# libnxz/power-gzip

Measured on AMD Instinct MI355X. Metric: GiB/s uncompressed in (deflate), real-data corpus in 64 KiB blocks, exact dynamic-Huffman table per block, higher is better.
Workload: dtype u8

## Files before the change

### power-gzip_amd/csrc/nxz_lz77.hip

```cpp
#include <hip/hip_runtime.h>
#include <type_traits>
#include <stdint.h>
#include "nxz_device.h"
#include "nxz_dhtgen_dev.h"
#include "nxz_dict.h"

__device__ unsigned long long *nxz_lz77_prof_buf = nullptr;
#define NXZ_GLOBAL NXZ_GLOBAL_AS
#ifdef NXZ_LZ77_PROF
#define WPROF_BEGIN() unsigned long long wp_ = prof ? clock64() : 0
#define WPROF_END(idx) do { if (prof) { const unsigned long long now_ = clock64(); wacc[(idx) - 16] += now_ - wp_; wp_ = now_; } } while (0)
#define PROF(idx) do { if (prof) { if (t == 0) { unsigned long long now_ = clock64(); profacc[idx] += (uint32_t)(now_ - tprev); tprev = now_; } } } while (0)
#define PCOUNT(idx, n) do { if (prof && lane == 0) atomicAdd(&profacc[idx], (uint32_t)(n)); } while (0)
#ifdef NXZ_LZ77_PROF2
#define PC2(idx, n) do { if (prof && lane == 0) __hip_atomic_fetch_add(&prof[32 + (idx)], (unsigned long long)(n), __ATOMIC_RELAXED, __HIP_MEMORY_SCOPE_AGENT); } while (0)
#else
#define PC2(idx, n) do { } while (0)
#endif
#else
#define PC2(idx, n) do { } while (0)
#define PCOUNT(idx, n) do { } while (0)
#define WPROF_BEGIN() do { } while (0)
#define WPROF_END(idx) do { } while (0)
#define PROF(idx) do { } while (0)
#endif

namespace nxzl77 {

constexpr int NT = 1024;
constexpr int HBITS = 13;
constexpr uint32_t HSIZE = 1u << HBITS;
constexpr uint32_t PTILE = 16384;
constexpr uint32_t PSEG = 16;
constexpr uint32_t NSEG = PTILE / PSEG;
constexpr uint32_t ETILE = 2048;
constexpr uint32_t LAZY_MAX = 32;
constexpr uint32_t MAXMATCH = 258;
constexpr uint32_t WINDOW = 32768;
constexpr uint32_t OPEN2 = 24;
constexpr uint32_t NOHASH = 0xFFFFu;
constexpr uint32_t SECOND_MIN_TOKENS = 3072;
constexpr uint32_t TEXT_HIGH_DIV = 16;
#ifndef NXZ_GROUP_ROUNDS
#define NXZ_GROUP_ROUNDS 24
#endif
#ifndef NXZ_GROUP_MIN
#define NXZ_GROUP_MIN 2
#endif
#ifndef NXZ_GROUP_GATE
#define NXZ_GROUP_GATE 3
#endif
constexpr uint32_t GROUP_ROUNDS = NXZ_GROUP_ROUNDS;
constexpr uint32_t GROUP_GATE = NXZ_GROUP_GATE;
constexpr uint32_t GROUP_MIN = NXZ_GROUP_MIN;
constexpr uint32_t C2_STRIDE = PTILE + 1024;

constexpr uint32_t OFF_IN    = 0;
constexpr uint32_t OFF_HEAD  = 65536 + 32;
constexpr uint32_t OFF_CAND  = OFF_HEAD + HSIZE * 4 + 256;
constexpr uint32_t OFF_MLEN  = OFF_CAND + PTILE * 2;
constexpr uint32_t OFF_SBITS = OFF_MLEN + PTILE;
constexpr uint32_t OFF_MBITS = OFF_SBITS + PTILE / 8;
constexpr uint32_t OFF_X     = OFF_MBITS + PTILE / 8;
constexpr uint32_t OFF_ENTRY = OFF_X + NSEG * 2;
constexpr uint32_t OFF_BITS  = OFF_ENTRY + NSEG * 2;
#ifndef NXZ_LQ_CAP
#define NXZ_LQ_CAP 128
#define NXZ_LQ_MIN 64
#endif
#ifndef NXZ_XQ_CAP
#define NXZ_XQ_CAP 120
#define NXZ_XQ_MIN 56
#endif
constexpr uint32_t LQ_CAP = NXZ_LQ_CAP, LQ_MIN = NXZ_LQ_MIN, XQ_CAP = NXZ_XQ_CAP, XQ_MIN = NXZ_XQ_MIN;
static_assert(LQ_MIN + 64 <= LQ_CAP && XQ_MIN + 64 <= XQ_CAP && LQ_CAP % 8 == 0 && XQ_CAP % 8 == 0, "a batch of 64 must fit behind what waits");
constexpr uint32_t BITS_BYTES = 16 * (LQ_CAP + XQ_CAP) * 2 + 2096 - NSEG * 4 < ETILE * 2 + 64 ? ETILE * 2 + 64 : 16 * (LQ_CAP + XQ_CAP) * 2 + 2096 - NSEG * 4;
constexpr uint32_t OFF_LQ    = OFF_X;
constexpr uint32_t OFF_DQ    = OFF_LQ;
constexpr uint32_t OFF_XQ    = OFF_LQ + 16 * LQ_CAP * 2;
constexpr uint32_t OFF_EB    = OFF_XQ + 16 * XQ_CAP * 2;
constexpr uint32_t EBO       = 32;
static_assert(OFF_EB % 16 == 0 && OFF_EB + 2096 <= OFF_BITS + BITS_BYTES, "match-phase carve");
constexpr uint32_t OFF_SCAN  = OFF_BITS + BITS_BYTES;
constexpr uint32_t OFF_HIST  = OFF_SCAN + 256;
constexpr uint32_t OFF_MISC  = OFF_HIST + 316 * 4;
constexpr uint32_t OFF_PROF  = OFF_MISC + 64;
constexpr uint32_t LDS_BYTES = OFF_PROF + 80;
static_assert(LDS_BYTES <= 163840, "LDS budget");
static_assert(OFF_HEAD % 16 == 0 && OFF_BITS % 16 == 0 && OFF_SCAN % 16 == 0, "alignment");

enum { M_NREC = 0, M_TOK0 = 1, M_HIGH = 2, M_DQ = 3, M_PROGRESS = 4, M_TICKET = 5, M_DEFER = 6, M_NEXT = 7, M_KEEP = 8, M_DEFER2 = 9, M_PREV = 12, M_JOBNO = 13 };
static_assert(M_TICKET == M_PROGRESS + 1 && M_DEFER == M_PROGRESS + 2, "cleared together");

__device__ __forceinline__ uint32_t lds_ld32(const uint32_t *inw, uint32_t r)
{
	uint32_t a = inw[r >> 2], b = inw[(r >> 2) + 1];
	return __builtin_amdgcn_alignbyte(b, a, r & 3);
}

__device__ __forceinline__ uint32_t hash4(uint32_t v) { return (v * 0x9E3779B1u) >> (32 - HBITS); }

__device__ __forceinline__ uint32_t equal16(const uint32_t *inw, uint32_t a, uint32_t b)
{
	const uint32_t aw = a >> 2, bw = b >> 2, as = a & 3, bs = b & 3;
	const uint32_t a0 = inw[aw], a1 = inw[aw + 1], a2 = inw[aw + 2], a3 = inw[aw + 3], a4 = inw[aw + 4];
	const uint32_t b0 = inw[bw], b1 = inw[bw + 1], b2 = inw[bw + 2], b3 = inw[bw + 3], b4 = inw[bw + 4];
	const uint32_t x0 = __builtin_amdgcn_alignbyte(a1, a0, as) ^ __builtin_amdgcn_alignbyte(b1, b0, bs);
	const uint32_t x1 = __builtin_amdgcn_alignbyte(a2, a1, as) ^ __builtin_amdgcn_alignbyte(b2, b1, bs);
	const uint32_t x2 = __builtin_amdgcn_alignbyte(a3, a2, as) ^ __builtin_amdgcn_alignbyte(b3, b2, bs);
	const uint32_t x3 = __builtin_amdgcn_alignbyte(a4, a3, as) ^ __builtin_amdgcn_alignbyte(b4, b3, bs);
	uint32_t n = 16;
	if (x3) n = 12 + ((uint32_t)__builtin_ctz(x3) >> 3);
	if (x2) n = 8 + ((uint32_t)__builtin_ctz(x2) >> 3);
	if (x1) n = 4 + ((uint32_t)__builtin_ctz(x1) >> 3);
	if (x0) n = (uint32_t)__builtin_ctz(x0) >> 3;
	return n;
}

__device__ __forceinline__ uint32_t gf_mul(uint32_t a, uint32_t b)
{
	uint32_t r = 0;
#pragma unroll 8
	for (int i = 0; i < 32; i++) {
		r ^= (b & 0x80000000u) ? a : 0;
		a = (a >> 1) ^ ((a & 1) ? 0xedb88320u : 0);
		b <<= 1;
	}
	return r;
}

constexpr uint32_t cgf_mul(uint32_t a, uint32_t b)
{
	uint32_t r = 0;
	for (int i = 0; i < 32; i++) {
		if (b & 0x80000000u) r ^= a;
		a = (a >> 1) ^ ((a & 1) ? 0xedb88320u : 0);
		b <<= 1;
	}
	return r;
}
struct PowTab { uint32_t v[1024]; };
constexpr PowTab make_pow()
{
	PowTab p{};
	uint32_t m = 0x00800000u;
	for (int k = 0; k < 6; k++) m = cgf_mul(m, m);
	p.v[0] = 0x80000000u;
	for (int i = 1; i < 1024; i++) p.v[i] = cgf_mul(p.v[i - 1], m);
	return p;
}
__device__ const PowTab CRC_POW = make_pow();
struct Pow8Tab { uint32_t v[65]; };
constexpr Pow8Tab make_pow8()
{
	Pow8Tab p{};
	p.v[0] = 0x80000000u;
	for (int i = 1; i <= 64; i++) p.v[i] = cgf_mul(p.v[i - 1], 0x00800000u);
	return p;
}
__device__ const Pow8Tab CRC_POW8 = make_pow8();

__device__ __forceinline__ uint32_t wave_incl_scan(uint32_t v, int lane)
{
#pragma unroll
	for (int o = 1; o < 64; o <<= 1) {
		uint32_t u = __shfl_up(v, o, 64);
		if (lane >= o) v += u;
	}
	return v;
}
// ... 274 lines not shown
	__syncthreads();
	uint32_t *w_ = win0 + par * (WW + 2);
	if (n == 0) {
		const uint32_t nfull = base_bits >> 5;
		for (uint32_t i = te; i < nfull; i += ENT)
			if (wordbase + i < cap_words) dstw[wordbase + i] = w_[i];
		const uint32_t keep = w_[nfull];
		__syncthreads();
		if (te == 0) w_[0] = keep;
		wordbase += nfull;
		base_bits &= 31;
		__syncthreads();
	}
	if (te == 0) {
		const uint32_t lt = lltab[256];
		uint32_t cc = 0;
		if (wordbase > cap_words) cc = NXZ_CC_TARGET_SPACE;
		if ((lt >> 16) == 0) cc = NXZ_CC_MISSING_CODE;
		if (tb->status) cc = NXZ_CC_INVALID_DHT;
		const uint64_t acc = (uint64_t)w_[0] | ((uint64_t)(lt & 0xffff) << base_bits);
		const uint32_t bits = base_bits + (lt >> 16);
		const uint64_t totbits = (uint64_t)wordbase * 32 + bits;
		const uint32_t tpbc = (uint32_t)((totbits + 7) >> 3);
		if (tpbc > job.dst_cap) cc = cc ? cc : NXZ_CC_TARGET_SPACE;
		if (cc != NXZ_CC_TARGET_SPACE && (uint64_t)wordbase * 4 + (bits + 7) / 8 <= job.dst_cap) {
			NXZ_GLOBAL uint8_t *o = (NXZ_GLOBAL uint8_t *)job.dst + (size_t)wordbase * 4;
			for (uint32_t b = 0; b < (bits + 7) / 8; b++) o[b] = (uint8_t)(acc >> (8 * b));
		}
		if (cc == 0 && tpbc > total) cc = NXZ_CC_TPBC_GT_SPBC;
		nxz_batch_result_t *r = results + bid;
		r->cc = cc;
		r->tpbc = cc == NXZ_CC_TARGET_SPACE ? 0 : tpbc;
		r->tebc = (uint32_t)(totbits & 7);
		r->sfbt = 0;
	}
}

__device__ __forceinline__ void post(uint8_t *lds, const nxz_batch_job_t *__restrict__ jobs, NXZ_GLOBAL uint8_t *scratch, nxz_batch_result_t *__restrict__ results,
				     bool have_cur, uint32_t cur_slot, uint32_t prev_plus1, uint32_t prev_slot, const int t)
{
	const NXZ_GLOBAL uint8_t *tabs = scratch + table_off(gridDim.x);
	const bool have_prev = prev_plus1 != 0;
	uint32_t nprev = 0;
	if (have_prev) {
		const uint32_t sl = jobs[prev_plus1 - 1].src_len, hl = jobs[prev_plus1 - 1].hist_len;
		nprev = sl - (hl < sl ? hl : sl);
	}
	nprev = (uint32_t)__builtin_amdgcn_readfirstlane((int)nprev);
	if (t < 64) {
		Credit cr{ have_prev ? encode_barriers(nprev) : 0u };
		if (have_cur) {
			uint32_t *hist = (uint32_t *)(lds + OFF_HIST);
			if (t == 0) hist[256] = 1;
			__builtin_amdgcn_fence(__ATOMIC_ACQ_REL, "wavefront");
			__builtin_amdgcn_wave_barrier();
			__builtin_amdgcn_s_setprio(3);
			nxzd::dhtgen_wave(lds + P_DHT, (const uint32_t *)hist, (nxz_dht_prepared_t *)(tabs + ((size_t)blockIdx.x * 2 + cur_slot) * sizeof(nxz_dht_prepared_t)),
					  (nxz_batch_dht_t *)nullptr, t, cr);
			__builtin_amdgcn_s_setprio(0);
		}
		while (cr.n) cr();
	} else if (have_prev) {
		encode(lds, jobs, prev_plus1 - 1, scratch + ((size_t)blockIdx.x * 2 + prev_slot) * NXZ_TOK_STRIDE,
		       (const NXZ_GLOBAL nxz_dht_prepared_t *)(tabs + ((size_t)blockIdx.x * 2 + prev_slot) * sizeof(nxz_dht_prepared_t)), results, t - 64);
	}
	__builtin_amdgcn_fence(__ATOMIC_RELEASE, "workgroup");
	__syncthreads();
	__builtin_amdgcn_fence(__ATOMIC_ACQUIRE, "workgroup");
}
}

template <bool COUNT, bool FUSED, bool GEN, bool DICT>
__device__ __forceinline__ void lz77_body(const nxz_batch_job_t *__restrict__ jobs,
					  uint8_t *__restrict__ tokens, uint16_t *__restrict__ cand2,
					  nxz_batch_result_t *__restrict__ results,
					  uint32_t *__restrict__ counts, uint32_t njobs, uint32_t *__restrict__ next_job,
					  const uint8_t *__restrict__ dict)
{
	__shared__ __attribute__((aligned(16))) uint8_t lds[LDS_BYTES];
	uint32_t *inw = (uint32_t *)(lds + OFF_IN);
	uint32_t *head = (uint32_t *)(lds + OFF_HEAD);
	uint16_t *cand = (uint16_t *)(lds + OFF_CAND);
	uint8_t *mlen = lds + OFF_MLEN;
	uint16_t *X = (uint16_t *)(lds + OFF_X);
	uint16_t *entry = (uint16_t *)(lds + OFF_ENTRY);
	uint32_t *sbits = (uint32_t *)(lds + OFF_SBITS);
	uint32_t *mbits = (uint32_t *)(lds + OFF_MBITS);
	uint32_t *tokbits = sbits;
	uint32_t *litbits = mbits;
	uint8_t *mark = lds + OFF_SBITS;
	uint16_t *jump = (uint16_t *)(lds + OFF_MBITS);
	uint32_t *bitbuf = (uint32_t *)(lds + OFF_BITS);
	uint32_t *scan = (uint32_t *)(lds + OFF_SCAN);
	uint32_t *hist = (uint32_t *)(lds + OFF_HIST);
	uint32_t *misc = (uint32_t *)(lds + OFF_MISC);
#ifdef NXZ_LZ77_PROF
	uint32_t *profacc = (uint32_t *)(lds + OFF_PROF);
#endif

#ifdef NXZ_LZ77_PROF
	NXZ_GLOBAL unsigned long long *prof = (NXZ_GLOBAL unsigned long long *)nxz_lz77_prof_buf;
#endif
	if constexpr (GEN) {
		if (threadIdx.x == 0) { misc[M_PREV] = 0; misc[M_JOBNO] = 0; }
		__syncthreads();
	}
	for (uint32_t bid = blockIdx.x; bid < njobs;) {
	if (next_job && threadIdx.x == 0) misc[M_NEXT] = gridDim.x + atomicAdd(next_job, 1u);
	int tid_ = threadIdx.x;
	asm volatile("" : "+v"(tid_));
	const int t = tid_, lane = t & 63, wave = t >> 6;
#ifdef NXZ_LZ77_PROF
	unsigned long long tprev = prof ? clock64() : 0;
	unsigned long long wacc[4] = { 0, 0, 0, 0 };
#endif
	const nxz_batch_job_t job = jobs[bid];
	const uint32_t total = job.src_len;
	const uint32_t h = job.hist_len < total ? job.hist_len : total;
	const uint32_t n = total - h;
	const uint32_t end = total;
	const NXZ_GLOBAL uint8_t *src = (const NXZ_GLOBAL uint8_t *)job.src;
	const uint32_t K1 = n ? (end - 1) >> 6 : 0;
	const uint32_t pw_slice = CRC_POW.v[(1022 - t) & 1023];
	const uint32_t pw_tail = CRC_POW8.v[n ? end - K1 * 64 : 0];

	{
		typedef uint32_t v4u __attribute__((ext_vector_type(4)));
		const NXZ_GLOBAL v4u *s4 = (const NXZ_GLOBAL v4u *)src;
		v4u *d4 = (v4u *)inw;
		uint32_t nfull = total >> 4;
		if constexpr (DICT) {
			const NXZ_GLOBAL v4u *w4 = (const NXZ_GLOBAL v4u *)dict;
			const uint32_t hq = h >> 4;
			for (uint32_t i = t; i < nfull; i += NT) d4[i] = i < hq ? w4[i] : s4[i];
		} else
		for (uint32_t i = t; i < nfull; i += NT) d4[i] = s4[i];
		uint32_t base = nfull << 4;
		for (uint32_t i = base + t; i < base + 48 && i < 65536 + 32; i += NT)
			lds[OFF_IN + i] = i < total ? src[i] : 0;
	}
	for (uint32_t i = t; i < HSIZE; i += NT) head[i] = 0;
	if (t < 316) hist[t] = 0;
	if (t < 16 && t != M_NEXT && !(GEN && (t == M_PREV || t == M_JOBNO))) misc[t] = FUSED && t == M_KEEP ? 3u : 0u;
#ifdef NXZ_LZ77_PROF
	if (t < 20) profacc[t] = 0;
#endif
	{
		uint32_t c = t & 255;
		for (int k = 0; k < 8 * ((t >> 8) + 1); k++) c = (c >> 1) ^ ((c & 1) ? 0xedb88320u : 0);
		bitbuf[t] = c;
	}
	__syncthreads();
	PROF(0);

	uint32_t out_crc, out_adler;
	{
		uint32_t *T = bitbuf;
		const uint32_t initx = job.in_crc ^ 0xffffffffu;
		const int sidx = (int)t - 1023 + (int)K1;
		uint32_t crc = 0, s1 = 0, sj = 0;
		if (n && sidx >= (int)(h >> 6)) {
			const uint4 *sp = (const uint4 *)(lds + OFF_IN + (uint32_t)sidx * 64);
			uint4 q[4] = { sp[0], sp[1], sp[2], sp[3] };
			uint32_t *w = (uint32_t *)q;
			const uint32_t a0 = (uint32_t)sidx * 64;
			if (a0 < h || a0 + 64 > end) {
#pragma unroll
				for (int k = 0; k < 16; k++)
					if (a0 + 4 * k < h || a0 + 4 * k + 4 > end) w[k] = 0;
			}
			uint32_t S = 0, Wt = 0;
#pragma unroll
			for (int k = 0; k < 16; k++) {
				S = __builtin_amdgcn_udot4(w[k], 0x01010101u, S, false);
				Wt = __builtin_amdgcn_udot4(w[k], 0x03020100u + 0x04040404u * k, Wt, false);
			}
			s1 = S;
			sj = S * (n + h - a0) - Wt;
			const uint32_t kfirst = a0 < h ? (h - a0) >> 2 : 0;
			if (a0 <= h && h < a0 + 64) {
				if (h + 4 <= end) {
					if (kfirst == 0) w[0] ^= initx;
					if (kfirst == 4) w[4] ^= initx;
					if (kfirst == 8) w[8] ^= initx;
					if (kfirst == 12) w[12] ^= initx;
				}
			}
			const uint32_t nd = a0 + 64 <= end ? 16 : (end - a0) >> 2;
#pragma unroll
			for (int k = 0; k < 16; k++) {
				const uint32_t c = crc ^ w[k];
				const uint32_t nc = T[768 + (c & 0xff)] ^ T[512 + ((c >> 8) & 0xff)] ^ T[256 + ((c >> 16) & 0xff)] ^ T[c >> 24];
				crc = (uint32_t)k < nd ? nc : crc;
			}
			if (t == 1023 && (end & 3)) {
				const uint32_t a = end & ~3u, nb = end & 3, i = a - h;
				const uint32_t v = inw[a >> 2] & ((1u << (8 * nb)) - 1);
				uint32_t b0 = v & 0xff, b1 = (v >> 8) & 0xff, b2 = (v >> 16) & 0xff;
				s1 += b0 + b1 + b2;
				sj += (b0 + b1 + b2) * (n - i) - (b1 + 2 * b2);
				if (i == 0) crc ^= initx;
				for (uint32_t k = 0; k < nb; k++) crc = T[(crc ^ (v >> (8 * k))) & 0xff] ^ (crc >> 8);
			}
		}
		uint32_t tailcrc = 0;
		if (t == 1023) { tailcrc = crc; crc = 0; }
		else if (crc) crc = gf_mul(crc, pw_slice);
		for (int o = 32; o > 0; o >>= 1) crc ^= __shfl_down(crc, o, 64);
		if (lane == 0) scan[wave] = crc;
		if (t == 1023) scan[50] = tailcrc;
		uint32_t a1 = s1, a2 = sj % 65521u;
		for (int o = 32; o > 0; o >>= 1) {
			a1 += __shfl_down(a1, o, 64);
			a2 += __shfl_down(a2, o, 64);
		}
		if (lane == 0) { scan[16 + wave] = a1; scan[32 + wave] = a2 % 65521u; }
		__syncthreads();
		if (wave == 0) {
			uint32_t c = lane < 16 ? scan[lane] : 0;
			uint32_t b1 = lane < 16 ? scan[16 + lane] : 0, b2 = lane < 16 ? scan[32 + lane] : 0;
			for (int o = 8; o > 0; o >>= 1) {
				c ^= __shfl_down(c, o, 64);
				b1 += __shfl_down(b1, o, 64);
				b2 += __shfl_down(b2, o, 64);
			}
			if (lane == 0) {
				c = n ? gf_mul(c, pw_tail) ^ scan[50] : initx;
				uint32_t ia = job.in_adler & 0xffff, ib = job.in_adler >> 16;
// ... 491 lines not shown
					lqn += (uint32_t)__popcll(m);
					PCOUNT(13, __popcll(m));
#endif
					__builtin_amdgcn_wave_barrier();
					WPROF_END(17);
					while (lqn >= (last ? 1u : LQ_MIN) || (last && xqn)) { stage2(lqn, last); lqn = lqn > 64 ? lqn - 64 : 0; }
					WPROF_END(18);
					rest &= rest - 1;
				}
				if (last) break;
			}
		}
		__syncthreads();
		PROF(12);
		for (uint32_t pc = wave; pc < 64; pc += NT / 64) {
			if (!((misc[pc & 32 ? M_DEFER2 : M_DEFER] >> (pc & 31)) & 1)) continue;
			const uint32_t ii = (pc << 8) + 255;
			if (cand[ii + 1] == cand[ii]) {
				if (lane == 0 && mlen[ii + 1] >= 5) kb[ii >> 5] |= 0x80000000u;
				continue;
			}
			const uint32_t r = h + tb0 + ii, q = r - cand[ii] - 1;
			const uint32_t maxlen = end - r < MAXMATCH ? end - r : MAXMATCH;
			uint32_t N = maxlen;
			for (uint32_t ob = 8; ob < maxlen; ob += 256) {
				const uint32_t o = ob + 4 * lane;
				const uint32_t x = o < maxlen ? lds_ld32(inw, q + o) ^ lds_ld32(inw, r + o) : 0;
				const unsigned long long mm = __ballot(x != 0);
				if (mm) {
					const int fl = __builtin_ctzll(mm);
					const uint32_t nn = ob + 4 * fl + ((uint32_t)__builtin_ctz(__shfl(x, fl, 64)) >> 3);
					N = nn < maxlen ? nn : maxlen;
					break;
				}
			}
			if (lane == 0) mlen[ii] = (uint8_t)(N - 3);
		}
		__syncthreads();
		PROF(10);
		const uint32_t p0 = (uint32_t)t * PSEG;
		{
			const uint32_t *eb = (const uint32_t *)(lds + OFF_EB);
			uint16_t *dq = (uint16_t *)(lds + OFF_DQ);
			const uint32_t e32 = p0 < tn ? lds_ld32(eb, 2 * t + EBO / 8) : 0;
			const bool runs = (e32 & (e32 >> 1) & (e32 >> 2) & (e32 >> 3) & 0xffff) != 0;
			const unsigned long long rm = __ballot(runs);
			if (rm) {
				uint32_t qb = 0;
				if (lane == 0) qb = atomicAdd(&misc[M_DQ], (uint32_t)__popcll(rm));
				qb = __builtin_amdgcn_readfirstlane(qb);
				if (runs) dq[qb + (uint32_t)__popcll(rm & ((1ull << lane) - 1))] = (uint16_t)t;
			}
		}
		if (p0 < tn) {
			const uint32_t kb16 = ((const uint16_t *)kb)[t];
			const uint32_t kbits = kb16 & ((const uint16_t *)vb)[t];
			if (kbits) {
				const uint4 mv = *(const uint4 *)(mlen + p0);
				uint32_t mw[4] = { mv.x, mv.y, mv.z, mv.w };
				uint32_t E = 0;
				if (kb16 >> 15) {
					const uint32_t lim = p0 + 16 + 272 < tn ? p0 + 16 + 272 : tn;
					uint32_t s0 = p0 + 16;
					asm volatile("" : "+v"(s0));
					const uint32_t T = first_zero(kb, s0, lim);
					E = T < lim ? T + mlen[T] + 3 : T + MAXMATCH;
				}
				const uint32_t room15 = end - (h + tb0 + p0 + 15);
#pragma unroll
				for (int j = 15; j >= 0; j--) {
					const uint32_t m = (mw[j >> 2] >> (8 * (j & 3))) & 0xff;
					E = (kb16 >> j) & 1 ? E : p0 + j + m + 3;
					const uint32_t room = room15 + (15 - j);
					uint32_t N = E - (p0 + j);
					N = N < room ? N : room;
					N = N < MAXMATCH ? N : MAXMATCH;
					if ((kbits >> j) & 1) mw[j >> 2] = (mw[j >> 2] & ~(0xffu << (8 * (j & 3)))) | ((N - 3) & 0xff) << (8 * (j & 3));
				}
				*(uint4 *)(mlen + p0) = make_uint4(mw[0], mw[1], mw[2], mw[3]);
			}
		}
		__syncthreads();
		PROF(11);
		for (uint32_t s = t; s < NSEG; s += NT) mark[s] = 0;
		{
			const uint32_t *eb = (const uint32_t *)(lds + OFF_EB);
			const uint16_t *dq = (const uint16_t *)(lds + OFF_DQ);
			const uint32_t qn = misc[M_DQ];
			for (uint32_t qi = t; qi < qn; qi += NT) {
				const uint32_t sg = dq[qi], q0 = sg * PSEG;
				const uint32_t e32 = lds_ld32(eb, 2 * sg + EBO / 8);
				const uint32_t e16 = e32 & 0xffff;
				const uint4 mv = *(const uint4 *)(mlen + q0);
				const uint4 c0 = ((const uint4 *)cand)[2 * sg], c1 = ((const uint4 *)cand)[2 * sg + 1];
				const uint32_t mw[4] = { mv.x, mv.y, mv.z, mv.w };
				uint32_t cw[8] = { c0.x, c0.y, c0.z, c0.w, c1.x, c1.y, c1.z, c1.w };
				uint32_t zb = 16;
				if (e16 >> 15) {
					uint32_t s0 = EBO + q0 + 16;
					asm volatile("" : "+v"(s0));
					zb = first_zero(eb, s0, s0 + 272) - EBO - q0;
				}
				const uint32_t r15 = h + tb0 + q0 + 15;
				uint32_t om[4] = { 0, 0, 0, 0 };
#pragma unroll
				for (int j = 15; j >= 0; j--) {
					const uint32_t i = q0 + j, r = r15 - (15 - j);
					const uint32_t room = end > r ? end - r : 0;
					const uint32_t ml = room < MAXMATCH ? room : MAXMATCH;
					const uint32_t mj = (mw[j >> 2] >> (8 * (j & 3))) & 0xff;
					uint32_t cj = (cw[j >> 1] >> (16 * (j & 1))) & 0xffff;
					const uint32_t NA = mj ? mj + 3 : 0;
					const uint32_t zmask = ~e16 & (0xffffu << j) & 0xffffu;
					const uint32_t zpos = zmask ? (uint32_t)__builtin_ctz(zmask) : zb;
					uint32_t NB = zpos - j;
					if (NB > ml) NB = ml;
					uint32_t len = NA;
					if (NB >= 4 && NB >= NA && i < tn) { len = NB; cj = 0; }
					om[j >> 2] |= (len ? len - 3 : 0) << (8 * (j & 3));
					cw[j >> 1] = (cw[j >> 1] & ~(0xffffu << (16 * (j & 1)))) | cj << (16 * (j & 1));
				}
				*(uint4 *)(mlen + q0) = make_uint4(om[0], om[1], om[2], om[3]);
				((uint4 *)cand)[2 * sg] = make_uint4(cw[0], cw[1], cw[2], cw[3]);
				((uint4 *)cand)[2 * sg + 1] = make_uint4(cw[4], cw[5], cw[6], cw[7]);
			}
		}
		__syncthreads();

		PROF(5);
		uint32_t sm0 = 0, sm1 = 0, sm2 = 0, sm3 = 0;
		uint32_t seg_next = 0, seg_nz = 0;
		uint32_t mm1 = 0, lit1 = 0;
		uint32_t lastd = 0;
		auto seg_m = [&](uint32_t k) -> uint32_t {
			const uint32_t a = (k & 8) ? sm2 : sm0, b = (k & 8) ? sm3 : sm1;
			const uint32_t w = (k & 4) ? b : a;
			const uint32_t v = (w >> (8 * (k & 3))) & 0xff;
			return (k & 16) ? seg_next : v;
		};
		auto seg_step = [&](uint32_t p, uint32_t limit, bool &is_match) -> uint32_t {
			const uint32_t k = p - p0, cur = seg_m(k);
			const uint32_t full = cur ? cur + 3 : 0;
			const uint32_t len = full < limit - p ? full : limit - p;
			is_match = false;
			if (full >= 4 && len >= 3) {
				if (len < lazy_max && p + 1 < limit) {
					uint32_t m2 = seg_m(k + 1);
					uint32_t l2 = m2 ? m2 + 3 : 0;
					if (l2 > limit - p - 1) l2 = limit - p - 1;
					if (l2 > len) return 1;
				}
				is_match = true;
				return len;
			}
			return 1;
		};
		if ((uint32_t)t < nseg) {
			{
				const uint4 mv = *(const uint4 *)(mlen + p0);
				sm0 = mv.x; sm1 = mv.y; sm2 = mv.z; sm3 = mv.w;
			}
			seg_next = p0 + 16 < tn ? mlen[p0 + 16] : 0;
			auto nz4 = [](uint32_t w) -> uint32_t {
				uint32_t x = (((w & 0x7f7f7f7fu) + 0x7f7f7f7fu) | w) & 0x80808080u;
				return (((x >> 7) * 0x00204081u) >> 21) & 0xf;
			};
			seg_nz = nz4(sm0) | nz4(sm1) << 4 | nz4(sm2) << 8 | nz4(sm3) << 12;
			uint32_t p = p0, stop = p + PSEG < tn ? p + PSEG : tn;
			uint32_t cov = 0;
			while (p < stop) {
				const uint32_t rest = seg_nz >> (p - p0);
				p += rest ? (uint32_t)__builtin_ctz(rest) : stop - p;
				bool m;
				const uint32_t adv = seg_step(p < stop ? p : p0, tn, m);
				const bool took = p < stop && m;
				mm1 |= took ? 1u << (p - p0) : 0;
				cov |= took ? (adv >= 16 ? 0xffffu : (1u << adv) - 1) << (p - p0) : 0;
				p += p < stop ? adv : 0;
			}
			lit1 = ~cov & (stop - p0 >= 16 ? 0xffffu : (1u << (stop - p0)) - 1);
			lastd = mm1 ? cand[p0 + 31 - (uint32_t)__builtin_clz(mm1)] : 0;
			if (p > stop && stop == tn) p = tn;
			X[t] = (uint16_t)(p < tn ? p : tn);
			jump[t] = (uint16_t)(p >= tn ? NSEG : p / PSEG);
		}
		if (t == 0) mark[0] = 1;
		__syncthreads();
		PROF(6);
		{
			uint16_t *ja = jump, *jb = entry;
			uint32_t j1 = (uint32_t)t < nseg ? ja[t] : NSEG;
			for (int k = 0; k < 5; k++) {
				if ((uint32_t)t < nseg) {
					const uint32_t j2 = j1 < NSEG ? ja[j1] : NSEG;
					const uint32_t j3 = j2 < NSEG ? ja[j2] : NSEG;
					const uint32_t j4 = j3 < NSEG ? ja[j3] : NSEG;
					if (mark[t]) {
						if (j1 < NSEG) mark[j1] = 1;
						if (j2 < NSEG) mark[j2] = 1;
						if (j3 < NSEG) mark[j3] = 1;
					}
					jb[t] = (uint16_t)j4;
					j1 = j4;
				}
				__syncthreads();
				uint16_t *tmp = ja; ja = jb; jb = tmp;
			}
		}
		bool entered = (uint32_t)t < nseg && mark[t];
		uint32_t myx = (uint32_t)t < nseg ? X[t] : 0;
		if (t == 0) entry[0] = 0;
		if (entered && myx < tn) entry[myx / PSEG] = (uint16_t)myx;
		__syncthreads();
		uint32_t mye = entered ? entry[t] : 0;
		sbits[t] = 0;
		__syncthreads();

		PROF(7);
		if (entered) {
			uint32_t p = mye;
			const uint32_t lim = myx;
			uint32_t lm = 0, mm = 0;
			const uint32_t vis1 = lit1 | mm1;
			const uint32_t jm = mm1 ? 31 - (uint32_t)__builtin_clz(mm1) : 0;
			const bool lastm = mm1 != 0 && (lit1 >> jm) <= 1u;
			while (p < lim) {
				const uint32_t k = p - p0;
				if (k < 16 && ((vis1 >> k) & 1)) {
					const uint32_t ms = mm1 & (0xffffffffu << k);
					lm |= lit1 & (0xffffffffu << k);
					mm |= ms;
					if (lim == tn && ms) {
						const uint32_t j = 31 - (uint32_t)__builtin_clz(ms), pl = p0 + j;
						if (pl + seg_m(j) + 3 > tn) mlen[pl] = (uint8_t)(tn - pl - 3);
					}
					break;
				}
				if (lastm && k > jm) {
					const uint32_t left = lim - p;
					if (left >= 3) {
						if (k < 32) mm |= 1u << k; else atomicOr(&tokbits[p >> 5], 1u << (p & 31));
						mlen[p] = (uint8_t)(left - 3);
						cand[p] = (uint16_t)lastd;
					} else {
						for (uint32_t q = p; q < lim; q++) {
							if (q - p0 < 32) lm |= 1u << (q - p0); else atomicOr(&litbits[q >> 5], 1u << (q & 31));
						}
					}
					break;
				}
				const uint32_t rest = (seg_nz | vis1) >> k;
				uint32_t run = rest ? (uint32_t)__builtin_ctz(rest) : 16 - k;
				if (run > lim - p) run = lim - p;
				if (run) {
					lm |= ((1u << run) - 1) << k;
					p += run;
					continue;
				}
				bool m;
				const uint32_t l = seg_step(p, lim, m);
				lm |= (m ? 0u : 1u) << k;
				mm |= (m ? 1u : 0u) << k;
				if (m) mlen[p] = (uint8_t)(l - 3);
				p += l;
			}
			const uint32_t sh = 16 * ((uint32_t)t & 1), wi = (uint32_t)t >> 1;
			const uint64_t lv = (uint64_t)lm << sh, mv = (uint64_t)mm << sh;
			if ((uint32_t)lv) atomicOr(&litbits[wi], (uint32_t)lv);
			if (lv >> 32) atomicOr(&litbits[wi + 1], (uint32_t)(lv >> 32));
			if ((uint32_t)mv) atomicOr(&tokbits[wi], (uint32_t)mv);
			if (mv >> 32) atomicOr(&tokbits[wi + 1], (uint32_t)(mv >> 32));
		}
		__syncthreads();
		PROF(8);
		if (tb0 == 0 && n > PTILE && t < 512) {
			uint32_t c = (uint32_t)__popc(litbits[t]) + (uint32_t)__popc(tokbits[t]);
			for (int o = 32; o > 0; o >>= 1) c += __shfl_down(c, o, 64);
			if (lane == 0) atomicAdd(&misc[M_TOK0], c);
		}

		if constexpr (FUSED) {
			Quad q[4] = { {0, 0, 0, 0}, {0, 0, 0, 0}, {0, 0, 0, 0}, {0, 0, 0, 0} };
			uint32_t nb = 0;
			if (p0 < tn) {
				const uint32_t tok16 = ((const uint16_t *)tokbits)[t], lit16 = ((const uint16_t *)litbits)[t];
				if (tok16 | lit16) {
					const uint4 bv = *(const uint4 *)(lds + OFF_IN + h + tb0 + p0);
					const uint4 mv = *(const uint4 *)(mlen + p0);
					const uint4 c0 = ((const uint4 *)cand)[2 * t], c1 = ((const uint4 *)cand)[2 * t + 1];
					q[0] = fx_quad(bv.x, lit16 & 15, tok16 & 15, mv.x, c0.x, c0.y);
					q[1] = fx_quad(bv.y, (lit16 >> 4) & 15, (tok16 >> 4) & 15, mv.y, c0.z, c0.w);
					q[2] = fx_quad(bv.z, (lit16 >> 8) & 15, (tok16 >> 8) & 15, mv.z, c1.x, c1.y);
					q[3] = fx_quad(bv.w, lit16 >> 12, tok16 >> 12, mv.w, c1.z, c1.w);
					nb = q[0].nb + q[1].nb + q[2].nb + q[3].nb;
				}
			}
			const uint32_t incl = wave_incl_scan(nb, lane);
			if (lane == 63) scan[wave] = incl;
			__syncthreads();
			uint32_t bitpos = obits + incl - nb, tilebits = 0;
#pragma unroll
			for (int w = 0; w < 16; w++) {
				const uint32_t sc = scan[w];
				if (w < wave) bitpos += sc;
				tilebits += sc;
			}
			uint32_t *win = (uint32_t *)(lds + OFF_CAND);
			const uint32_t tot = obits + tilebits, nfull = tot >> 5;
			for (uint32_t i = t; i < (nfull + 8) / 4 + 1; i += NT) ((uint4 *)win)[i] = make_uint4(0, 0, 0, 0);
			__syncthreads();
			if (t == 0) atomicOr(&win[0], misc[M_KEEP]);
			fx_emit(win, q[0], bitpos);
			fx_emit(win, q[1], bitpos + q[0].nb);
			fx_emit(win, q[2], bitpos + q[0].nb + q[1].nb);
			fx_emit(win, q[3], bitpos + q[0].nb + q[1].nb + q[2].nb);
			__syncthreads();
			for (uint32_t i = t; i < nfull; i += NT)
				if (wordbase + i < cap_words) dstw[wordbase + i] = win[i];
			if (t == 0) misc[M_KEEP] = win[nfull];
			wordbase += nfull;
			obits = tot & 31;
			__syncthreads();
		} else
		{
			const uint32_t tok16 = p0 < tn ? ((const uint16_t *)tokbits)[t] : 0;
			const uint32_t nm = (uint32_t)__popc(tok16);
			uint32_t incl = wave_incl_scan(nm, lane);
			if (lane == 63) scan[wave] = incl;
			const uint32_t recbase = misc[M_NREC];
			__syncthreads();
			uint32_t rank = recbase + incl - nm, tot = 0;
#pragma unroll
			for (int w = 0; w < 16; w++) {
				const uint32_t sc = scan[w];
				if (w < wave) rank += sc;
				tot += sc;
			}
			for (uint32_t mbits_ = tok16; mbits_; mbits_ &= mbits_ - 1) {
				const uint32_t p = p0 + (uint32_t)__builtin_ctz(mbits_);
				const uint32_t l3 = mlen[p], d = cand[p];
				if (rank < NXZ_TOK_MAXREC) g_rec[rank] = l3 | (d << 8);
				rank++;
				if (COUNT) {
					uint32_t le = l3 < 8 ? 0 : (29 - (uint32_t)__builtin_clz(l3 | 8));
					const uint32_t ls = l3 == 255 ? 28 : (le << 2) + (l3 >> le);
					const uint32_t de = d < 4 ? 0 : (30 - (uint32_t)__builtin_clz(d | 4));
					const uint32_t ds = d < 4 ? d : 2 * de + 2 + ((d >> de) & 1);
					atomicAdd(&hist[257 + ls], 1u);
					atomicAdd(&hist[286 + ds], 1u);
				}
			}
			if (COUNT && p0 < tn) {
				const uint32_t lit16 = ((const uint16_t *)litbits)[t];
				if (lit16) {
					const uint4 bv = *(const uint4 *)(lds + OFF_IN + h + tb0 + p0);
					for (uint32_t lb = lit16; lb; lb &= lb - 1) {
						const uint32_t k = (uint32_t)__builtin_ctz(lb);
						const uint32_t a = (k & 8) ? bv.z : bv.x, b = (k & 8) ? bv.w : bv.y;
						const uint32_t w = (k & 4) ? b : a;
						atomicAdd(&hist[(w >> (8 * (k & 3))) & 0xff], 1u);
					}
				}
			}
			{
				const uint32_t nwords = (tn + 31) >> 5, i = (uint32_t)t & 511;
				if (i < nwords) {
					if (t < 512) g_lit[(tb0 >> 5) + i] = litbits[i];
					else g_tok[(tb0 >> 5) + i] = tokbits[i];
				}
			}
			__syncthreads();
			if (t == 0) misc[M_NREC] = recbase + tot;
		}
		PROF(9);
	}

	if (t == 0) {
		nxz_batch_result_t r;
		r.cc = 0; r.tpbc = 0; r.tebc = 0;
		r.spbc = DICT ? n : total; r.crc = out_crc; r.adler = out_adler; r.subc = 0;
		r.sfbt = misc[M_NREC];
		if constexpr (FUSED) {
			const uint64_t acc = misc[M_KEEP];
			const uint32_t bits = obits + 7;
			const uint64_t totbits = (uint64_t)wordbase * 32 + bits;
			const uint32_t tpbc = (uint32_t)((totbits + 7) >> 3);
			uint32_t cc = wordbase > cap_words || tpbc > job.dst_cap ? NXZ_CC_TARGET_SPACE : 0;
			if (!cc) {
				NXZ_GLOBAL uint8_t *o = (NXZ_GLOBAL uint8_t *)job.dst + (size_t)wordbase * 4;
				for (uint32_t b = 0; b < (bits + 7) / 8; b++) o[b] = (uint8_t)(acc >> (8 * b));
				if (tpbc > total) cc = NXZ_CC_TPBC_GT_SPBC;
			}
			r.cc = cc; r.tpbc = cc == NXZ_CC_TARGET_SPACE ? 0 : tpbc; r.tebc = (uint32_t)(totbits & 7); r.sfbt = 0;
		}
		results[bid] = r;
	}
#ifdef NXZ_LZ77_PROF
	if (prof) {
		if (lane == 0) for (int k = 0; k < 4; k++) atomicAdd(&profacc[16 + k], (uint32_t)wacc[k]);
		__syncthreads();
		if (t < 20) __hip_atomic_fetch_add(&prof[t], (unsigned long long)profacc[t], __ATOMIC_RELAXED, __HIP_MEMORY_SCOPE_AGENT);
	}
#endif
	if (COUNT && (!GEN || counts)) {
		__syncthreads();
		if (t < 316) counts[(size_t)bid * 316 + t] = (t == 256) ? 1u : hist[t];
	}
	if constexpr (GEN) {
		__builtin_amdgcn_fence(__ATOMIC_RELEASE, "workgroup");
		__syncthreads();
		__builtin_amdgcn_fence(__ATOMIC_ACQUIRE, "workgroup");
		const uint32_t prev = (uint32_t)__builtin_amdgcn_readfirstlane((int)misc[M_PREV]);
		gen::post(lds, jobs, (NXZ_GLOBAL uint8_t *)tokens, results, true, gslot, prev, gslot ^ 1u, t);
		if (t == 0) { misc[M_PREV] = bid + 1; misc[M_JOBNO] = misc[M_JOBNO] + 1; }
	}
	__syncthreads();
	const uint32_t drawn = next_job ? misc[M_NEXT] : bid + gridDim.x;
	__syncthreads();
	bid = drawn;
	}
	if constexpr (GEN) {
		const uint32_t prev = (uint32_t)__builtin_amdgcn_readfirstlane((int)misc[M_PREV]);
		const uint32_t slot = ((uint32_t)__builtin_amdgcn_readfirstlane((int)misc[M_JOBNO]) & 1u) ^ 1u;
		if (prev) gen::post(lds, jobs, (NXZ_GLOBAL uint8_t *)tokens, results, false, 0, prev, slot, (int)threadIdx.x);
	}
}

template <bool COUNT, bool FUSED = false, bool GEN = false>
__global__ __launch_bounds__(NT) void lz77_kernel(const nxz_batch_job_t *__restrict__ jobs,
						  uint8_t *__restrict__ tokens, uint16_t *__restrict__ cand2,
						  nxz_batch_result_t *__restrict__ results,
						  uint32_t *__restrict__ counts, uint32_t njobs, uint32_t *__restrict__ next_job)
{
	lz77_body<COUNT, FUSED, GEN, false>(jobs, tokens, cand2, results, counts, njobs, next_job, nullptr);
}

template <bool COUNT, bool FUSED = false, bool GEN = false>
__global__ __launch_bounds__(NT) void lz77_dict_kernel(const nxz_batch_job_t *__restrict__ jobs,
						       uint8_t *__restrict__ tokens, uint16_t *__restrict__ cand2,
						       nxz_batch_result_t *__restrict__ results,
						       uint32_t *__restrict__ counts, uint32_t njobs, uint32_t *__restrict__ next_job,
						       const uint8_t *__restrict__ dict)
{
	lz77_body<COUNT, FUSED, GEN, true>(jobs, tokens, cand2, results, counts, njobs, next_job, dict);
}

__global__ __launch_bounds__(256) void dict_jobs_kernel(const nxz_batch_job_t *__restrict__ in, uint32_t n, uint32_t W, nxz_batch_job_t *__restrict__ out)
{
	const uint32_t i = blockIdx.x * 256 + threadIdx.x;
	if (i >= n) return;
	nxz_batch_job_t j = in[i];
	if (nxz_dict_job_fits(W, j.src_len, j.hist_len)) {
		j.src = (const uint8_t *)((uintptr_t)j.src - W);
		j.src_len += W; j.hist_len = W;
	} else { j.src_len = 0; j.hist_len = 0; j.dst_cap = 0; }
	out[i] = j;
}
__global__ __launch_bounds__(256) void dict_finish_kernel(const nxz_batch_job_t *__restrict__ in, uint32_t n, uint32_t W, nxz_batch_result_t *__restrict__ results)
{
	const uint32_t i = blockIdx.x * 256 + threadIdx.x;
	if (i >= n) return;
	if (nxz_dict_job_fits(W, in[i].src_len, in[i].hist_len)) return;
	nxz_batch_result_t r = {};
	r.cc = NXZ_CC_INVALID_OP;
	results[i] = r;
}

}

extern "C" int nxz_launch_dict_jobs(const nxz_batch_job_t *in, size_t n, uint32_t W, nxz_batch_job_t *out, hipStream_t stream)
{
	if (!n) return 0;
	hipLaunchKernelGGL(nxzl77::dict_jobs_kernel, dim3((unsigned)((n + 255) / 256)), dim3(256), 0, stream, in, (uint32_t)n, W, out);
	return (int)hipGetLastError();
}
extern "C" int nxz_launch_dict_finish(const nxz_batch_job_t *in, size_t n, uint32_t W, nxz_batch_result_t *results, hipStream_t stream)
{
	if (!n) return 0;
	hipLaunchKernelGGL(nxzl77::dict_finish_kernel, dim3((unsigned)((n + 255) / 256)), dim3(256), 0, stream, in, (uint32_t)n, W, results);
	return (int)hipGetLastError();
}

extern "C" int nxz_lz77_prof_set(unsigned long long *buf)
{
// ... 52 lines not shown
```

Before: 105.5.

## Resolve segment entry chain with wavefront permutes instead of LDS pointer doubling

Replaces the LDS-based pointer-jumping over segment jump tables, which took five rounds each ending in a block barrier and used mark/entry arrays, with per-wavefront hop resolution. Within a wavefront it uses ds_bpermute/ds_permute, then chains the exits of earlier wavefronts serially through a small shared exit table read with readlane. This removes several workgroup barriers and LDS round trips from the greedy-parse segment resolution step. In exchange there is a serial loop over up to 15 earlier wavefronts per thread and an assumption that a match hops at most a bounded number of segments. It also adds profiling points that compile away by default.

```diff
diff --git a/power-gzip_amd/csrc/nxz_lz77.hip b/power-gzip_amd/csrc/nxz_lz77.hip
--- a/power-gzip_amd/csrc/nxz_lz77.hip
+++ b/power-gzip_amd/csrc/nxz_lz77.hip
@@ -63,6 +63,10 @@
 constexpr uint32_t OFF_MBITS = OFF_SBITS + PTILE / 8;
 constexpr uint32_t OFF_X     = OFF_MBITS + PTILE / 8;
 constexpr uint32_t OFF_ENTRY = OFF_X + NSEG * 2;
+constexpr uint32_t MAXHOP = (PSEG - 1 + MAXMATCH) / PSEG;
+constexpr uint32_t NEXIT = 18;
+constexpr uint32_t XNONE = NSEG * PSEG;
+static_assert(PSEG == 16 && MAXHOP <= NEXIT && MAXHOP < 64 && 3 * NEXIT <= 64 && 16 * NEXIT * 2 <= NSEG * 2 && XNONE <= 0xffff, "exits of a wavefront");
 constexpr uint32_t OFF_BITS  = OFF_ENTRY + NSEG * 2;
 #ifndef NXZ_LQ_CAP
 #define NXZ_LQ_CAP 128
@@ -85,7 +89,11 @@
 constexpr uint32_t OFF_HIST  = OFF_SCAN + 256;
 constexpr uint32_t OFF_MISC  = OFF_HIST + 316 * 4;
 constexpr uint32_t OFF_PROF  = OFF_MISC + 64;
+#ifdef NXZ_LZ77_PROF
+constexpr uint32_t LDS_BYTES = OFF_PROF + 96;
+#else
 constexpr uint32_t LDS_BYTES = OFF_PROF + 80;
+#endif
 static_assert(LDS_BYTES <= 163840, "LDS budget");
 static_assert(OFF_HEAD % 16 == 0 && OFF_BITS % 16 == 0 && OFF_SCAN % 16 == 0, "alignment");
 
@@ -526,14 +534,11 @@
 	uint32_t *head = (uint32_t *)(lds + OFF_HEAD);
 	uint16_t *cand = (uint16_t *)(lds + OFF_CAND);
 	uint8_t *mlen = lds + OFF_MLEN;
-	uint16_t *X = (uint16_t *)(lds + OFF_X);
-	uint16_t *entry = (uint16_t *)(lds + OFF_ENTRY);
+	uint16_t *xtab = (uint16_t *)(lds + OFF_X);
 	uint32_t *sbits = (uint32_t *)(lds + OFF_SBITS);
 	uint32_t *mbits = (uint32_t *)(lds + OFF_MBITS);
 	uint32_t *tokbits = sbits;
 	uint32_t *litbits = mbits;
-	uint8_t *mark = lds + OFF_SBITS;
-	uint16_t *jump = (uint16_t *)(lds + OFF_MBITS);
 	uint32_t *bitbuf = (uint32_t *)(lds + OFF_BITS);
 	uint32_t *scan = (uint32_t *)(lds + OFF_SCAN);
 	uint32_t *hist = (uint32_t *)(lds + OFF_HIST);
@@ -587,7 +592,7 @@
 	if (t < 316) hist[t] = 0;
 	if (t < 16 && t != M_NEXT && !(GEN && (t == M_PREV || t == M_JOBNO))) misc[t] = FUSED && t == M_KEEP ? 3u : 0u;
 #ifdef NXZ_LZ77_PROF
-	if (t < 20) profacc[t] = 0;
+	if (t < 24) profacc[t] = 0;
 #endif
 	{
 		uint32_t c = t & 255;
@@ -1245,7 +1250,7 @@
 		}
 		__syncthreads();
 		PROF(11);
-		for (uint32_t s = t; s < NSEG; s += NT) mark[s] = 0;
+		sbits[t] = 0;
 		{
 			const uint32_t *eb = (const uint32_t *)(lds + OFF_EB);
 			const uint16_t *dq = (const uint16_t *)(lds + OFF_DQ);
@@ -1295,6 +1300,7 @@
 		uint32_t seg_next = 0, seg_nz = 0;
 		uint32_t mm1 = 0, lit1 = 0;
 		uint32_t lastd = 0;
+		uint32_t xval = XNONE;
 		auto seg_m = [&](uint32_t k) -> uint32_t {
 			const uint32_t a = (k & 8) ? sm2 : sm0, b = (k & 8) ? sm3 : sm1;
 			const uint32_t w = (k & 4) ? b : a;
@@ -1344,40 +1350,56 @@
 			lit1 = ~cov & (stop - p0 >= 16 ? 0xffffu : (1u << (stop - p0)) - 1);
 			lastd = mm1 ? cand[p0 + 31 - (uint32_t)__builtin_clz(mm1)] : 0;
 			if (p > stop && stop == tn) p = tn;
-			X[t] = (uint16_t)(p < tn ? p : tn);
-			jump[t] = (uint16_t)(p >= tn ? NSEG : p / PSEG);
-		}
-		if (t == 0) mark[0] = 1;
-		__syncthreads();
+			xval = p < tn ? p : XNONE;
+		}
 		PROF(6);
+		bool entered;
+		uint32_t myx, mye;
 		{
-			uint16_t *ja = jump, *jb = entry;
-			uint32_t j1 = (uint32_t)t < nseg ? ja[t] : NSEG;
-			for (int k = 0; k < 5; k++) {
-				if ((uint32_t)t < nseg) {
-					const uint32_t j2 = j1 < NSEG ? ja[j1] : NSEG;
-					const uint32_t j3 = j2 < NSEG ? ja[j2] : NSEG;
-					const uint32_t j4 = j3 < NSEG ? ja[j3] : NSEG;
-					if (mark[t]) {
-						if (j1 < NSEG) mark[j1] = 1;
-						if (j2 < NSEG) mark[j2] = 1;
-						if (j3 < NSEG) mark[j3] = 1;
-					}
-					jb[t] = (uint16_t)j4;
-					j1 = j4;
-				}
-				__syncthreads();
-				uint16_t *tmp = ja; ja = jb; jb = tmp;
-			}
-		}
-		bool entered = (uint32_t)t < nseg && mark[t];
-		uint32_t myx = (uint32_t)t < nseg ? X[t] : 0;
-		if (t == 0) entry[0] = 0;
-		if (entered && myx < tn) entry[myx / PSEG] = (uint16_t)myx;
-		__syncthreads();
-		uint32_t mye = entered ? entry[t] : 0;
-		sbits[t] = 0;
-		__syncthreads();
+			int ln = lane;
+			asm volatile("" : "+v"(ln));
+			const uint32_t base = (uint32_t)(t - ln), wend = base + 64;
+			auto hop = [&](uint32_t x) -> uint32_t {
+				const uint32_t sg = x >> 4;
+				const uint32_t v = (uint32_t)__builtin_amdgcn_ds_bpermute((int)((sg < wend ? sg - base : (uint32_t)ln) << 2), (int)x);
+				return sg < wend ? v : x;
+			};
+			uint32_t x = xval;
+#pragma unroll
+			for (int k = 0; k < 6; k++) x = hop(x);
+			if (ln < (int)NEXIT) xtab[wave * NEXIT + lane] = (uint16_t)x;
+			__syncthreads();
+			uint32_t xt[5];
+#pragma unroll
+			for (int r = 0; r < 5; r++) xt[r] = ln < 3 * (int)NEXIT ? xtab[r * 3 * NEXIT + ln] : 0;
+			const uint32_t wv = (uint32_t)__builtin_amdgcn_readfirstlane(wave);
+			uint32_t e = 0;
+#pragma unroll
+			for (int w = 0; w < 15; w++) {
+				if ((uint32_t)w < wv) {
+					const uint32_t off = e < XNONE ? (e >> 4) - 64 * w : 0;
+					const uint32_t nx = (uint32_t)__builtin_amdgcn_readlane((int)xt[w / 3], (int)__builtin_amdgcn_readfirstlane(off + NEXIT * (w % 3)));
+					e = e < XNONE ? nx : XNONE;
+				}
+			}
+			const uint32_t le = (e >> 4) - base;
+			bool m = (uint32_t)ln == le;
+			x = xval;
+#pragma unroll
+			for (int k = 0; k < 6; k++) {
+				const uint32_t sg = x >> 4;
+				const bool push = m && sg < wend;
+				const uint32_t got = (uint32_t)__builtin_amdgcn_ds_permute((int)(push ? (sg - base) << 2 : 0), push ? 1 : 0);
+				m = m || (ln != 0 && got != 0);
+				x = hop(x);
+			}
+			const uint32_t sg = xval >> 4;
+			const bool push = m && sg < wend;
+			const uint32_t got = (uint32_t)__builtin_amdgcn_ds_permute((int)(push ? (sg - base) << 2 : 0), (int)(push ? xval : 0));
+			entered = m && (uint32_t)t < nseg;
+			myx = xval < tn ? xval : tn;
+			mye = !entered ? 0 : (uint32_t)ln == le ? e : got;
+		}
 
 		PROF(7);
 		if (entered) {
@@ -1499,6 +1521,7 @@
 				if (w < wave) rank += sc;
 				tot += sc;
 			}
+			PROF(20);
 			for (uint32_t mbits_ = tok16; mbits_; mbits_ &= mbits_ - 1) {
 				const uint32_t p = p0 + (uint32_t)__builtin_ctz(mbits_);
 				const uint32_t l3 = mlen[p], d = cand[p];
@@ -1513,6 +1536,7 @@
 					atomicAdd(&hist[286 + ds], 1u);
 				}
 			}
+			PROF(21);
 			if (COUNT && p0 < tn) {
 				const uint32_t lit16 = ((const uint16_t *)litbits)[t];
 				if (lit16) {
@@ -1525,6 +1549,7 @@
 					}
 				}
 			}
+			PROF(22);
 			{
 				const uint32_t nwords = (tn + 31) >> 5, i = (uint32_t)t & 511;
 				if (i < nwords) {
@@ -1562,7 +1587,7 @@
 	if (prof) {
 		if (lane == 0) for (int k = 0; k < 4; k++) atomicAdd(&profacc[16 + k], (uint32_t)wacc[k]);
 		__syncthreads();
-		if (t < 20) __hip_atomic_fetch_add(&prof[t], (unsigned long long)profacc[t], __ATOMIC_RELAXED, __HIP_MEMORY_SCOPE_AGENT);
+		if (t < 24) __hip_atomic_fetch_add(&prof[t], (unsigned long long)profacc[t], __ATOMIC_RELAXED, __HIP_MEMORY_SCOPE_AGENT);
 	}
 #endif
 	if (COUNT && (!GEN || counts)) {
```

Measured after the change: 106.3 (median of 6 runs). Within noise of the previous version (+0.8%).
